# MarioPasc/MU-Diff

Measured on AMD Instinct MI355X. Metric: 256x256 slices/sec (4-step dual-gen reverse), higher is better.
Workload: dtype f32 (convs/attention: fp16 hi+lo split MFMA x3; 3x3 convs that fill the chip: fp16 hi.hi + e4m3 cross terms; fp32 accumulate); 1 GPU; BASELINE config 3 (BraTS-shaped test-split batches of 32; model and slice shapes of config 2): 4-step dual-generator sampling, 256x256, nf=64, ch_mult 1-2-4, 32 slices per GPU per step, batch-sharded over 1 GPU(s), weights replicated; batch=32, hipgraph=True

## Files before the change

include/mudiff_hip.h:

```cpp
#ifndef MUDIFF_HIP_H
#define MUDIFF_HIP_H

#include <stdint.h>

#ifdef __cplusplus
extern "C" {
#endif

#define MUD_OK 0
#define MUD_ERR_ARG 1
#define MUD_ERR_LAUNCH 2
#define MUD_ERR_UNSUPPORTED 3

#define MUD_ACT_NONE 0
#define MUD_ACT_SIGMOID 1
#define MUD_ACT_TANH 2
#define MUD_ACT_SILU 3
#define MUD_ACT_LRELU 4

#define MUD_PRO_NONE 0
#define MUD_PRO_AFFINE 1
#define MUD_PRO_AFFINE_SILU 2
#define MUD_PRO_LRELU 3

// ... 25 lines not shown
  float* out; int ldo;
  int maxdim;
} mud_mlp_args;
int mud_mlp_chain(const mud_mlp_args* a, void* stream);
int mud_mlp_chains(const mud_mlp_args* a, int n, void* stream);

int64_t mud_gn_ws_bytes(int B, int64_t HW, int C, int G);
int mud_gn_scale_shift(const float* x, int B, int64_t HW, int C, int ld, int G, float eps,
                       const float* gamma, const float* beta, int64_t g_bstride,
                       float* scale, float* shift, int ld_ss, float* mean_rstd ,
                       void* ws, void* stream);
int mud_gn_scale_shift_from_sums(const double* sums, int sums_ld, int B, int C, int G, double count, float eps,
                                 const float* gamma, const float* beta, int64_t g_bstride,
                                 float* scale, float* shift, int ld_ss, void* stream);
int mud_channel_mean(const float* x, int B, int64_t HW, int C, int ld, float* out, int ldo, void* ws, void* stream);

typedef struct mud_conv_args {
  const float* x;  int B, H, W, Cin, ldx;
  const void* w;   int64_t w_bstride;
  int ks, stride, pad;
  const float* pro_scale; const float* pro_shift; int pro_ld; int pro_mode;
  const float* bias;
  const float* bias2; int bias2_ld;
  const float* res; int ldr;
  float out_scale; int act;
  const float* emul; int ld_emul;
  const float* egate; int ld_egate;
  const float* eother; int ld_eother;
  float* out; int Cout, ldo;
  int sub2;
  double* stats; int stats_ld;
  int emul_cout;
  const double* gn_sums; int gn_sums_ld;
  int gn_G; float gn_eps; double gn_count;
  const float* gn_gamma; const float* gn_beta;
  int64_t gn_bstride;
  void* splitk_ws; int64_t splitk_ws_bytes;
  unsigned* splitk_counters; int splitk_ncounters;
  const void* skip_w; const float* skip_bias; float* skip_out; int skip_ldo;
  int prec; int w_exp;
} mud_conv_args;

int mud_conv2d_direct(const mud_conv_args* a, void* stream);

int64_t mud_packed_weight_bytes(int ks, int Cin, int Cout);
int mud_pack_weights(const float* src, int64_t s_tap, int64_t s_ci, int64_t s_co, int64_t src_bstride,
                     int ks, int Cin, int Cout, int nbatch, void* dst, void* stream);
int mud_pack_weights_prec(const float* src, int64_t s_tap, int64_t s_ci, int64_t s_co, int64_t src_bstride,
                          int ks, int Cin, int Cout, int nbatch, int prec, int w_exp, void* dst, void* stream);
int64_t mud_packed_weight_bytes_prec(int ks, int Cin, int Cout, int prec);
int mud_conv2d_mfma(const mud_conv_args* a, void* stream);
int mud_conv2d_mfma_prec_supported(const mud_conv_args* a, int prec);
int64_t mud_conv2d_mfma_splitk_bytes(const mud_conv_args* a);

typedef struct mud_census_args {
  const float* x; int B, H, W, C, ldx;
  const float* pro_scale; const float* pro_shift; int pro_ld; int pro_mode;
} mud_census_args;
typedef struct mud_census_out {
  uint64_t n, n_over, n_under, n_fp16_over, amax_bits;
} mud_census_out;
int mud_e4m3_census(const mud_census_args* a, mud_census_out* out, void* stream);

int mud_upfirdn2d(const float* in, int64_t planes, int H, int W, const float* kernel, int kh, int kw,
                  int up_x, int up_y, int down_x, int down_y, int pad_x0, int pad_x1, int pad_y0, int pad_y1,
                  float* out, void* stream);
int mud_fir_nhwc(const float* x, int B, int H, int W, int C, int ldx, const float* kernel_host, int kh, int kw,
                 int up, int down, int pad0, int pad1,
// ... 118 lines not shown
```

mu-diff_amd/backbones/layerspp.py:

```python
import numpy as np
import torch
import torch.nn as nn

from mudiff_hip import ops, precision
from mudiff_hip.ops import (ACT_NONE, ACT_SILU, INV_SQRT2, PRO_AFFINE, PRO_AFFINE_SILU, View)

from . import dense_layer, layers, up_or_down_sampling

conv1x1 = layers.ddpm_conv1x1
conv3x3 = layers.ddpm_conv3x3
NIN = layers.NIN
default_init = layers.default_init
dense = dense_layer.dense

FIR_K = (1, 3, 3, 1)


def _groups(c):
    return min(c // 4, 32)


def use_mfma(cin, cout):
    return cin % 4 == 0 and cin >= 8

# ... 270 lines not shown
        self.dropout = dropout

    def _prepare(self):
        d = dict(c0=ConvParam(self.Conv_0), c1=ConvParam(self.Conv_1))
        if hasattr(self, 'Conv_2'):
            d['c2'] = ConvParam(self.Conv_2)
            if self.up:
                d['c2'].bias = None
                d['c1'].bias = (self.Conv_1.bias.detach() + self.Conv_2.bias.detach()).contiguous()
        return d

    def run(self, x: View, style0, style1, tbias, out: View = None, arena=None):
        if self.dropout and self.training:
            raise NotImplementedError('dropout > 0 in training mode is not part of the inference path')
        p = self.prepared()
        fused = False
        gn0 = self.GroupNorm_0.scale_shift(x, style0)
        sc0, sh0 = (gn0, None) if isinstance(gn0, ops.LazyGN) else gn0
        if self.up:
            kk, up, down, pad = up_or_down_sampling.fir_params('up' if self.fir else 'naive_up', self.fir_kernel)
            h_in, _ = ops.fir_nhwc(x, kk, up, down, pad, pro=(sc0, sh0, PRO_AFFINE_SILU), want_h=True, want_x=False)
            x_skip, _ = ops.fir_nhwc(p['c2'](x), kk, up, down, pad)
            h = p['c0'](h_in, bias2=tbias, arena=arena)
        elif self.down:
            kk, up, down, pad = up_or_down_sampling.fir_params('down' if self.fir else 'naive_down', self.fir_kernel)
            h_in, x_skip = ops.fir_nhwc(x, kk, up, down, pad, pro=(sc0, sh0, PRO_AFFINE_SILU), want_h=True, want_x=True)
            h = p['c0'](h_in, bias2=tbias, arena=arena)
        else:
            x_skip = x
            fused = 'c2' in p and p['c0'].mfma and p['c2'].mfma and ops.fused_skip_ok(x, self.out_ch, PRO_AFFINE_SILU)
            if fused:
                x_skip = View.empty(x.B, x.H, x.W, self.out_ch, x.device)
                h = p['c0'](x, pro=(sc0, sh0, PRO_AFFINE_SILU), bias2=tbias, arena=arena, skip=(p['c2'].w, p['c2'].bias, x_skip))
            else:
                h = p['c0'](x, pro=(sc0, sh0, PRO_AFFINE_SILU), bias2=tbias, arena=arena)
        gn1 = self.GroupNorm_1.scale_shift(h, style1)
        sc1, sh1 = (gn1, None) if isinstance(gn1, ops.LazyGN) else gn1
        if 'c2' in p and not self.up and not fused:
            x_skip = p['c2'](x_skip)
        return p['c1'](h, pro=(sc1, sh1, PRO_AFFINE_SILU), res=x_skip, out_scale=INV_SQRT2 if self.skip_rescale else 1.0, out=out)

    def forward(self, x, temb=None, zemb=None):
        st0 = ops.dense(zemb, self.GroupNorm_0.style.weight.detach(), self.GroupNorm_0.style.bias.detach())
        st1 = ops.dense(zemb, self.GroupNorm_1.style.weight.detach(), self.GroupNorm_1.style.bias.detach())
        tb = None
        if temb is not None:
            tb = ops.dense(temb, self.Dense_0.weight.detach(), self.Dense_0.bias.detach(), act_in=ACT_SILU)
        return self.run(View.from_nchw(x), st0, st1, tb).to_nchw()


class ConvFeatBlock(nn.Module, _Prepared):

    def __init__(self, act, in_ch=None, out_ch=None, zemb_dim=256):
        super().__init__()
        self.conv1 = conv3x3(in_ch, out_ch)
# ... 48 lines not shown
        return self.run(View.from_nchw(x), st).to_nchw()


class ConvBlock_GAP(nn.Module, _Prepared):

    def __init__(self, act, in_ch=None, out_ch=None, zemb_dim=256):
        super().__init__()
        self.conv1 = conv3x3(in_ch, out_ch)
        self.group_norm = GroupNorm_Conv(min(out_ch // 4, 32), out_ch)
        self.act = act
        self.conv2 = conv3x3(out_ch, out_ch)
        self.adaptive_gap = nn.AdaptiveAvgPool2d(1)
        self.fc = dense(out_ch, zemb_dim)

    def _prepare(self):
        return dict(c1=ConvParam(self.conv1), c2=ConvParam(self.conv2))

    def run(self, x: View, arena=None):
        p = self.prepared()
        h = p['c1'](x, arena=arena)
        gn = self.group_norm.scale_shift(h)
        sc, sh = (gn, None) if isinstance(gn, ops.LazyGN) else gn
        h = p['c2'](h, pro=(sc, sh, PRO_AFFINE_SILU))
        gap = ops.channel_mean(h)
        assert gap.shape[1] == self.fc.in_features, f'GAP vector {gap.shape[1]} != fc.in_features {self.fc.in_features}'
        return ops.dense(gap, self.fc.weight.detach(), self.fc.bias.detach())

    def forward(self, x):
        return self.run(View.from_nchw(x))


class GaussianFourierProjection(nn.Module):

    def __init__(self, embedding_size=256, scale=1.0):
# ... 50 lines not shown
```

mu-diff_amd/csrc/conv_direct.hip:

```cpp
#include "mud_common.h"
#include <stdlib.h>

template <int VO, int VI>
__global__ __launch_bounds__(256) void k_conv_direct(mud_conv_args a, int Ho, int Wo, int co_groups) {
  extern __shared__ __attribute__((aligned(16))) char smem_raw[];
  float* st_lds = (float*)smem_raw;
  const int b = blockIdx.y;
  if (a.stats) {
    for (int i = threadIdx.x; i < 2 * a.Cout; i += 256) st_lds[i] = 0.f;
    __syncthreads();
  }
  const unsigned total = (unsigned)Ho * (unsigned)Wo * (unsigned)co_groups;
  const unsigned nthreads = gridDim.x * blockDim.x;
  const unsigned stride = (nthreads / (unsigned)co_groups) * (unsigned)co_groups;
  const unsigned first = blockIdx.x * blockDim.x + threadIdx.x;
  const int cg = (int)(first % (unsigned)co_groups);
  float ssum[VO], ssq[VO];
#pragma unroll
  for (int j = 0; j < VO; ++j) ssum[j] = ssq[j] = 0.f;
  for (uint64_t idx64 = first; first < stride && idx64 < total; idx64 += stride) {
    const unsigned p = (unsigned)idx64 / (unsigned)co_groups;
    const int oy = (int)(p / (unsigned)Wo);
    const int ox = (int)(p - (unsigned)oy * (unsigned)Wo);
    const int co = cg * VO;
// ... 206 lines not shown
      if (a.res) v += a.res[opix * a.ldr + j];
      a.out[opix * a.ldo + j] = mud_act(v * a.out_scale, a.act);
    }
  }
}

extern "C" int mud_conv2d_direct(const mud_conv_args* ap, void* stream) {
  MUD_REQUIRE(ap, "mud_conv2d_direct: null args");
  const mud_conv_args a = *ap;
  MUD_REQUIRE(a.x && a.w && a.out, "mud_conv2d_direct: null pointer");
  MUD_REQUIRE(a.B >= 0 && a.H > 0 && a.W > 0 && a.Cin > 0 && a.Cout > 0 && a.ks >= 1 && a.stride >= 1 && a.pad >= 0,
              "mud_conv2d_direct: bad sizes");
  MUD_REQUIRE(a.ldx >= a.Cin && a.ldo >= a.Cout, "mud_conv2d_direct: ld smaller than C");
  MUD_REQUIRE(a.pro_mode == MUD_PRO_NONE || a.pro_mode == MUD_PRO_LRELU || (a.pro_scale && a.pro_shift && a.pro_ld >= a.Cin), "mud_conv2d_direct: prologue arrays missing");
  MUD_REQUIRE(!a.res || a.ldr >= a.Cout, "mud_conv2d_direct: bad residual view");
  const int Ho = (a.H + 2 * a.pad - a.ks) / a.stride + 1, Wo = (a.W + 2 * a.pad - a.ks) / a.stride + 1;
  MUD_REQUIRE(Ho > 0 && Wo > 0, "mud_conv2d_direct: empty output");
  if (a.B == 0) return MUD_OK;
  const bool vo4 = a.Cout % 4 == 0 && a.ldo % 4 == 0 && mud_aligned16(a.out) && mud_aligned16(a.w) && (a.w_bstride % 16 == 0);
  const bool vi4 = a.Cin % 4 == 0 && a.ldx % 4 == 0 && mud_aligned16(a.x);
  const int co_groups = vo4 ? a.Cout / 4 : a.Cout;
  if (a.Cin == 1 && a.ks == 3 && ((a.stride == 1 && a.pad == 1) || (a.stride == 2 && a.pad == 0)) && vo4 && !a.emul && !a.egate && co_groups <= 256 && a.pro_mode == MUD_PRO_NONE && a.w_bstride == 0 &&
      (!a.res || (a.ldr % 4 == 0 && mud_aligned16(a.res))) && (!a.bias || mud_aligned16(a.bias)) &&
      (!a.bias2 || (a.bias2_ld % 4 == 0 && mud_aligned16(a.bias2)))) {
    MUD_REQUIRE(a.B <= 65535 && (!a.stats || a.stats_ld >= a.Cout), "mud_conv2d_direct: bad batch / stats view");
    const int spb = 256 / co_groups, strips_per_row = (int)mud_cdiv(Wo, HEAD_PIX);
    int64_t blocks = mud_cdiv((int64_t)Ho * strips_per_row, spb);
    if (blocks > 256 * 16) blocks = 256 * 16;
    if (a.stats) {
      static const int cap = getenv("MUD_HEAD_CAP") ? atoi(getenv("MUD_HEAD_CAP")) : 0;
// ... 46 lines not shown
```

mu-diff_amd/csrc/conv_mfma.hip:

```cpp
#include "mud_common.h"
#include <stdlib.h>
#include <type_traits>
#include <utility>

typedef int i32x4 __attribute__((ext_vector_type(4)));
typedef int i32x8 __attribute__((ext_vector_type(8)));
typedef _Float16 f16x4 __attribute__((ext_vector_type(4)));
typedef _Float16 f16x8 __attribute__((ext_vector_type(8)));

typedef mud_h16x4 h16x4;
typedef mud_h16x8 h16x8;
__device__ __forceinline__ int cm_e4m3x4(f32x4 v, float scale) {
  v = v * scale;
#pragma unroll
  for (int e = 0; e < 4; ++e) v[e] = __builtin_amdgcn_fmed3f(v[e], -448.0f, 448.0f);
  int p = __builtin_amdgcn_cvt_pk_fp8_f32(v[0], v[1], 0, false);
  return __builtin_amdgcn_cvt_pk_fp8_f32(v[2], v[3], p, true);
}
#define CM_BN 64
#define CM_BPLANE (CM_BN * 32)
#define CM_BSTEP (2 * CM_BPLANE)
#define CM_PIX 80
#define CM_GN_MAXC 1024
#define CM_GN_BYTES (2 * CM_GN_MAXC * 4)
// ... 320 lines not shown
        *(i32x4*)(smem + loff[j] + 64) = i32x4{0, 0, 0, 0};
        *(i32x4*)(smem + G::BUF + loff[j] + 64) = i32x4{0, 0, 0, 0};
      }
    }
  }
  dma_b(kc0 * G::NG);
  dma_b2(kc0);
  fetch_raw(kc0);

  const int emul_lim = a.emul_cout > 0 ? a.emul_cout : a.Cout;
  const bool vec = ((a.Cout | a.ldo | emul_lim | (a.res ? a.ldr : 0) | (a.emul ? a.ld_emul : 0) | (a.egate ? (a.ld_egate | a.ld_eother) : 0)) & 3) == 0 &&
                   mud_dev_aligned16(a.out) && (!a.res || mud_dev_aligned16(a.res)) && (!a.emul || mud_dev_aligned16(a.emul)) &&
                   (!a.egate || (mud_dev_aligned16(a.egate) && mud_dev_aligned16(a.eother)));
  const bool slab_mode = KS == 3 && nsplit > 1 && fin.counters != nullptr;
  const bool res_in_acc = !DUAL && KS == 3 && a.res != nullptr && !a.sub2 && nsplit == 1;
  if (res_in_acc) {
#pragma unroll
    for (int n = 0; n < 2; ++n) {
      const int co = (nt * WN + wn) * CM_BN + n * 32 + r;
#pragma unroll
      for (int m = 0; m < MT; ++m) {
        const int gy = ty0 + wm * MT + m;
#pragma unroll
        for (int reg = 0; reg < 16; ++reg) {
          const int gx = tx0 + (reg & 3) + 8 * (reg >> 2) + 4 * hh;
          const bool ok = gy < a.H && gx < a.W && co < a.Cout;
          acc[m][n][reg] = ok ? a.res[(((int64_t)b * a.H + gy) * a.W + gx) * a.ldr + co] : 0.f;
        }
      }
    }
  }
// ... 947 lines not shown
  if (a.ks != 3 || a.sub2 || (a.pro_mode != MUD_PRO_NONE && a.pro_mode != MUD_PRO_AFFINE_SILU)) return false;
  if (a.skip_w && a.pro_mode != MUD_PRO_AFFINE_SILU) return false;
  const int v = cm_variant3(a, nullptr);
  return v == CMV_8X2 || v == CMV_16X1 || v == CMV_8X1R;
}
extern "C" int mud_conv2d_mfma_prec_supported(const mud_conv_args* ap, int prec) {
  if (!ap || ap->B <= 0 || ap->H <= 0 || ap->W <= 0 || ap->Cin <= 0 || ap->Cout <= 0) return 0;
  if (prec == MUD_PREC_16X3) return ap->ks == 1 || ap->ks == 3;
  if (prec == MUD_PREC_16X1)
    return ap->ks == 3 && ap->pro_mode >= MUD_PRO_NONE && ap->pro_mode <= MUD_PRO_LRELU && (!ap->skip_w || ap->pro_mode == MUD_PRO_AFFINE_SILU);
  mud_conv_args a = *ap;
  a.prec = prec;
  return prec == MUD_PREC_FP8X && cm_fp8x_built(a);
}

extern "C" int mud_conv2d_mfma(const mud_conv_args* ap, void* stream) {
  MUD_REQUIRE(ap, "mud_conv2d_mfma: null args");
  mud_conv_args a = *ap;
  MUD_REQUIRE(a.x && a.w && a.out, "mud_conv2d_mfma: null pointer");
  MUD_REQUIRE((a.ks == 1 || a.ks == 3) && a.stride == 1 && a.pad == a.ks / 2, "mud_conv2d_mfma: only ks in {1,3}, stride 1, pad ks/2 (got ks=%d stride=%d pad=%d)", a.ks, a.stride, a.pad);
  MUD_REQUIRE(a.B >= 0 && a.H > 0 && a.W > 0 && a.Cin > 0 && a.Cout > 0, "mud_conv2d_mfma: bad sizes");
  MUD_REQUIRE(a.Cin % 4 == 0 && a.ldx % 4 == 0 && a.ldx >= a.Cin && mud_aligned16(a.x), "mud_conv2d_mfma: needs Cin%%4==0 (Cin=%d), ldx%%4==0 (ldx=%d), 16-byte aligned x", a.Cin, a.ldx);
  MUD_REQUIRE((int64_t)a.H * a.W * a.ldx < 0x7fffffffLL, "mud_conv2d_mfma: one image must stay below 2^31 elements");
  MUD_REQUIRE(mud_aligned16(a.w) && a.w_bstride % 16 == 0, "mud_conv2d_mfma: packed weights must be 16-byte aligned");
  MUD_REQUIRE(a.ldo >= a.Cout && (!a.res || a.ldr >= a.Cout), "mud_conv2d_mfma: bad output/residual view");
  MUD_REQUIRE(!a.stats || a.stats_ld >= a.Cout, "mud_conv2d_mfma: bad stats view");
  MUD_REQUIRE(!a.sub2 || (a.ks == 3 && (a.H & 1) && (a.W & 1)), "mud_conv2d_mfma: sub2 needs ks == 3 and odd H, W");
  MUD_REQUIRE(a.emul_cout >= 0 && a.emul_cout <= a.Cout, "mud_conv2d_mfma: emul_cout out of range");
  MUD_REQUIRE((!a.emul || a.ld_emul >= (a.emul_cout > 0 ? a.emul_cout : a.Cout)) && (!a.egate || (a.eother && a.ld_egate >= a.Cout && a.ld_eother >= a.Cout)), "mud_conv2d_mfma: bad emul / egate / eother view");
  MUD_REQUIRE(a.pro_mode >= MUD_PRO_NONE && a.pro_mode <= MUD_PRO_LRELU, "mud_conv2d_mfma: unknown prologue mode %d", a.pro_mode);
// ... 8 lines not shown
    MUD_REQUIRE(a.pro_scale && a.pro_shift && a.pro_ld >= a.Cin && a.pro_ld % 4 == 0 && mud_aligned16(a.pro_scale) && mud_aligned16(a.pro_shift),
                "mud_conv2d_mfma: prologue arrays missing or misaligned");
    MUD_REQUIRE(a.Cin <= CM_GN_MAXC, "mud_conv2d_mfma: a launch with prologue arrays takes Cin <= %d (the kernels keep them in LDS; Cin=%d)", CM_GN_MAXC, a.Cin);
  } else {
    a.pro_scale = a.pro_shift = a.x;
    a.pro_ld = 0;
    a.gn_sums = nullptr;
  }
  if (a.skip_w) {
    MUD_REQUIRE(a.ks == 3 && a.pro_mode == MUD_PRO_AFFINE_SILU && !a.res && !a.sub2 && !a.emul && !a.egate,
                "mud_conv2d_mfma: the fused skip conv needs ks == 3, the AFFINE_SILU prologue and a plain epilogue");
    MUD_REQUIRE(a.skip_out && a.Cin <= 512 && a.Cout % 4 == 0 && a.skip_ldo >= a.Cout && a.skip_ldo % 4 == 0 && a.ldo % 4 == 0 &&
                mud_aligned16(a.skip_w) && mud_aligned16(a.skip_out) && mud_aligned16(a.out),
                "mud_conv2d_mfma: fused skip conv needs Cin <= 512, Cout %% 4 == 0 and aligned float4 output rows (Cin=%d Cout=%d)", a.Cin, a.Cout);
  }
  MUD_REQUIRE(a.prec == MUD_PREC_16X3 || a.prec == MUD_PREC_FP8X || a.prec == MUD_PREC_16X1, "mud_conv2d_mfma: unknown arithmetic plan prec=%d", a.prec);
  MUD_REQUIRE(a.prec != MUD_PREC_16X1 || a.ks == 3, "mud_conv2d_mfma: MUD_PREC_16X1 is built for ks == 3 only (got ks=%d)", a.ks);
  MUD_REQUIRE(a.prec != MUD_PREC_FP8X || (cm_fp8x_built(a) && a.w_exp >= -100 && a.w_exp <= 100),
              "mud_conv2d_mfma: MUD_PREC_FP8X is not built for this launch (ask mud_conv2d_mfma_prec_supported first; the weights were packed for it and cannot be read by another plan)");
  if (a.B == 0) return MUD_OK;
  hipStream_t s = (hipStream_t)stream;
#ifdef MUD_EXPERIMENT_WS
  if (cm_ws_wanted(a)) return cm_ws_dispatch(a, s);
#endif
  if (a.prec == MUD_PREC_FP8X) {
    const int v8 = cm_variant3(a, nullptr);
    if (v8 == CMV_8X1R) return a.pro_mode == MUD_PRO_NONE ? cm_launch_pro<3, 1, 8, 1, MUD_PRO_NONE, false, MUD_PREC_FP8X>(a, s) : cm_launch_pro<3, 1, 8, 1, MUD_PRO_AFFINE_SILU, false, MUD_PREC_FP8X>(a, s);
    const bool x2 = v8 == CMV_8X2;
    if (a.skip_w) return x2 ? cm_launch_pro<3, 2, 4, 2, MUD_PRO_AFFINE_SILU, true, MUD_PREC_FP8X>(a, s) : cm_launch_pro<3, 2, 8, 1, MUD_PRO_AFFINE_SILU, true, MUD_PREC_FP8X>(a, s);
    if (a.pro_mode == MUD_PRO_NONE) return x2 ? cm_launch_pro<3, 2, 4, 2, MUD_PRO_NONE, false, MUD_PREC_FP8X>(a, s) : cm_launch_pro<3, 2, 8, 1, MUD_PRO_NONE, false, MUD_PREC_FP8X>(a, s);
// ... 44 lines not shown
```

mu-diff_amd/mudiff_hip/__init__.py:

```python
from __future__ import annotations

import ctypes as C
import os

import torch

_HERE = os.path.dirname(os.path.abspath(__file__))
_SHIPPED = os.path.join(_HERE, 'libmudiff_hip.so')
_LIB_PATH = os.environ.get('MUDIFF_HIP_LIB', _SHIPPED)
_lib = None
PREC_16X3, PREC_FP8X, PREC_16X1 = 0, 1, 2

ACT_NONE, ACT_SIGMOID, ACT_TANH, ACT_SILU, ACT_LRELU = 0, 1, 2, 3, 4
PRO_NONE, PRO_AFFINE, PRO_AFFINE_SILU, PRO_LRELU = 0, 1, 2, 3


class MudiffHipError(RuntimeError):
    pass


class ConvArgs(C.Structure):
    _fields_ = [
        ('x', C.c_void_p), ('B', C.c_int), ('H', C.c_int), ('W', C.c_int), ('Cin', C.c_int), ('ldx', C.c_int),
        ('w', C.c_void_p), ('w_bstride', C.c_int64),
# ... 2 lines not shown
        ('bias', C.c_void_p),
        ('bias2', C.c_void_p), ('bias2_ld', C.c_int),
        ('res', C.c_void_p), ('ldr', C.c_int),
        ('out_scale', C.c_float), ('act', C.c_int),
        ('emul', C.c_void_p), ('ld_emul', C.c_int), ('egate', C.c_void_p), ('ld_egate', C.c_int), ('eother', C.c_void_p), ('ld_eother', C.c_int),
        ('out', C.c_void_p), ('Cout', C.c_int), ('ldo', C.c_int),
        ('sub2', C.c_int),
        ('stats', C.c_void_p), ('stats_ld', C.c_int),
        ('emul_cout', C.c_int),
        ('gn_sums', C.c_void_p), ('gn_sums_ld', C.c_int), ('gn_G', C.c_int), ('gn_eps', C.c_float), ('gn_count', C.c_double),
        ('gn_gamma', C.c_void_p), ('gn_beta', C.c_void_p), ('gn_bstride', C.c_int64),
        ('splitk_ws', C.c_void_p), ('splitk_ws_bytes', C.c_int64),
        ('splitk_counters', C.c_void_p), ('splitk_ncounters', C.c_int),
        ('skip_w', C.c_void_p), ('skip_bias', C.c_void_p), ('skip_out', C.c_void_p), ('skip_ldo', C.c_int),
        ('prec', C.c_int), ('w_exp', C.c_int),
    ]


MLP_MAX_LAYERS = 6


class MlpArgs(C.Structure):
    _fields_ = [
        ('x', C.c_void_p), ('ldx', C.c_int), ('B', C.c_int),
        ('nlayers', C.c_int), ('dims', C.c_int * (MLP_MAX_LAYERS + 1)),
        ('W', C.c_void_p * MLP_MAX_LAYERS), ('b', C.c_void_p * MLP_MAX_LAYERS),
        ('pixel_norm', C.c_int), ('act', C.c_int), ('act_last', C.c_int),
        ('out', C.c_void_p), ('ldo', C.c_int), ('maxdim', C.c_int),
    ]

# ... 23 lines not shown
_SIGNATURES = {
    'mud_version': (C.c_int, []),
    'mud_last_error': (C.c_char_p, []),
    'mud_build_flags': (C.c_char_p, []),
    'mud_posterior_sample': (_I, [_P, _P, _P, _P, _P, _P, _P, _P, _I, _P, _I, _L, _P]),
    'mud_q_sample': (_I, [_P, _P, _P, _I, _P, _P, _I, _P, _I, _L, _P]),
    'mud_timestep_embedding': (_I, [_P, _P, _I, _I, _F, _P]),
    'mud_pixel_norm': (_I, [_P, _P, _I, _I, _P]),
    'mud_dense': (_I, [_P, _I, _P, _P, _P, _I, _I, _I, _I, _I, _I, _P]),
    'mud_mlp_chain': (_I, [C.POINTER(MlpArgs), _P]),
    'mud_mlp_chains': (_I, [C.POINTER(MlpArgs), _I, _P]),
    'mud_gn_ws_bytes': (_L, [_I, _L, _I, _I]),
    'mud_gn_scale_shift': (_I, [_P, _I, _L, _I, _I, _I, _F, _P, _P, _L, _P, _P, _I, _P, _P, _P]),
    'mud_gn_scale_shift_from_sums': (_I, [_P, _I, _I, _I, _I, C.c_double, _F, _P, _P, _L, _P, _P, _I, _P]),
    'mud_channel_mean': (_I, [_P, _I, _L, _I, _I, _P, _I, _P, _P]),
    'mud_conv2d_direct': (_I, [C.POINTER(ConvArgs), _P]),
    'mud_packed_weight_bytes': (_L, [_I, _I, _I]),
    'mud_pack_weights': (_I, [_P, _L, _L, _L, _L, _I, _I, _I, _I, _P, _P]),
    'mud_pack_weights_prec': (_I, [_P, _L, _L, _L, _L, _I, _I, _I, _I, _I, _I, _P, _P]),
    'mud_packed_weight_bytes_prec': (_L, [_I, _I, _I, _I]),
    'mud_conv2d_mfma': (_I, [C.POINTER(ConvArgs), _P]),
    'mud_conv2d_mfma_prec_supported': (_I, [C.POINTER(ConvArgs), _I]),
    'mud_conv2d_mfma_splitk_bytes': (_L, [C.POINTER(ConvArgs)]),
    'mud_upfirdn2d': (_I, [_P, _L, _I, _I, _P, _I, _I, _I, _I, _I, _I, _I, _I, _I, _I, _P, _P]),
    'mud_fir_nhwc': (_I, [_P, _I, _I, _I, _I, _I, C.POINTER(C.c_float), _I, _I, _I, _I, _I, _I, _P, _P, _I, _I, _P, _I, _P, _I, _P]),
    'mud_minibatch_stddev': (_I, [_P, _I, _L, _I, _I, _I, _P, _P]),
    'mud_attention_supported': (_I, [_I]),
    'mud_attention_ws_bytes': (_L, [_I, _I, _I]),
    'mud_attention': (_I, [_P, _I, _I, _I, _I, _F, _P, _I, _P, _P]),
    'mud_softmax_rows': (_I, [_P, _L, _I, _I, _P]),
    'mud_mul': (_I, [_P, _I, _P, _I, _P, _I, _L, _I, _P]),
    'mud_gate_mix': (_I, [_P, _I, _P, _I, _P, _I, _P, _I, _I, _L, _I, _P, _I, _P]),
    'mud_fourier_embedding': (_I, [_P, _P, _P, _I, _I, _P]),
    'mud_resize_bilinear': (_I, [_P, _L, _I, _I, _I, _I, _P, _P]),
    'mud_affine_clamp': (_I, [_P, _L, _F, _F, _F, _F, _P, _P]),
    'mud_e4m3_census': (_I, [C.POINTER(CensusArgs), _P, _P]),
    'mud_value_range_ws_bytes': (_L, []),
    'mud_value_range': (_I, [_P, _L, _P, _L, _P, _P, _P]),
# ... 95 lines not shown
```

mu-diff_amd/mudiff_hip/ops.py:

```python
from __future__ import annotations

import collections
import ctypes as C
import math
import os

import numpy as np
import torch

from . import (ACT_LRELU, ACT_NONE, ACT_SIGMOID, ACT_SILU, ACT_TANH, PREC_16X1, PREC_16X3, PREC_FP8X, PRO_AFFINE, PRO_AFFINE_SILU, PRO_LRELU,
               PRO_NONE, ConvArgs, MudiffHipError, check, load, ptr, require_gpu)


DETERMINISTIC = os.environ.get('MUD_DETERMINISTIC', '0') == '1'


class StatsArena:

    def __init__(self, device, chunk_doubles=1 << 18):
        self.device, self.chunk = device, chunk_doubles
        self.buf, self.used = None, 0

    def take(self, B, C):
        if DETERMINISTIC:
# ... 317 lines not shown
def conv3x3_would_split_k(x: View, cout):
    a = ConvArgs()
    a.x, a.B, a.H, a.W, a.Cin, a.ldx, a.ks, a.stride, a.pad = x.ptr, x.B, x.H, x.W, x.C, x.ld, 3, 1, 1
    a.out, a.Cout, a.ldo = x.ptr, cout, (cout + 3) & ~3
    return load().mud_conv2d_mfma_splitk_bytes(C.byref(a)) > 0


FUSE_SKIP_SPLIT = os.environ.get('MUD_FUSE_SKIP_SPLIT', '1') != '0'


def fused_skip_ok(x: View, cout, pro_mode):
    return (FUSE_SKIP and pro_mode == PRO_AFFINE_SILU and x.C % 4 == 0 and 8 <= x.C <= 512 and cout % 4 == 0
            and (FUSE_SKIP_SPLIT or not conv3x3_would_split_k(x, cout)))


def resolve_pro(pro):
    if pro is not None and isinstance(pro[0], LazyGN):
        sc, sh = pro[0].tensors()
        return (sc, sh, pro[2])
    return pro


def channel_mean(x: View):
    lib = load()
    HW = x.H * x.W
    ws = _workspace(x.device, lib.mud_gn_ws_bytes(x.B, HW, x.C, x.C))
    out = torch.empty(x.B, x.C, device=x.device, dtype=torch.float32)
    _launch('channel_mean', x.device, lib.mud_channel_mean, x.ptr, x.B, HW, x.C, x.ld, ptr(out), x.C, ptr(ws), STREAM, nbytes=4.0 * x.npix * x.C)
    return out


def pack_weights(src, s_tap, s_ci, s_co, ks, Cin, Cout, nbatch=1, src_bstride=0, src_offset=0, prec=PREC_16X3, w_exp=0):
    lib = load()
    require_gpu(src)
    nbytes = lib.mud_packed_weight_bytes_prec(ks, Cin, Cout, prec)
    if nbytes < 0:
        raise MudiffHipError(f'pack_weights: plan {prec} has no packed form for ks={ks}')
    dst = torch.empty(nbatch, nbytes, device=src.device, dtype=torch.uint8)
    _launch('pack_weights', src.device, lib.mud_pack_weights_prec, C.c_void_p(src.data_ptr() + 4 * src_offset), s_tap, s_ci, s_co, src_bstride, ks, Cin, Cout,
            nbatch, prec, w_exp, ptr(dst), STREAM)
    return dst


# ... 62 lines not shown
    if PREC_PLAN == 'fp16':
        return PREC_16X1 if conv_prec_supported(x, cout, pro_mode, PREC_16X1, skip=skip, sub2=sub2) else PREC_16X3
    if PREC_PLAN != 'all' and not fp8x_pays(x.B, x.H, x.W, x.C, cout):
        return PREC_16X3
    return PREC_FP8X if conv_prec_supported(x, cout, pro_mode, PREC_FP8X, skip=skip, sub2=sub2) else PREC_16X3


Launch = collections.namedtuple('Launch', 'layer ks mfma prec shape sub2 skip pro')


RECORD = None


def conv(x: View, w, ks, Cout, *, mfma, stride=1, pad=None, pro=None, bias=None, bias2=None, res: View = None,
         out_scale=1.0, act=ACT_NONE, out: View = None, w_bstride=0, arena=None, sub2=False, emul: View = None, gate=None, emul_cout=0,
         skip=None, prec=PREC_16X3, w_exp=0, layer=None):
    if RECORD is not None:
        if torch.cuda.is_current_stream_capturing():
            raise RuntimeError('precision.launch_record() is eager only: the launch is being captured into a graph')
        RECORD.append(Launch(layer, ks, bool(mfma), prec, (x.B, x.H, x.W, x.C, Cout), bool(sub2), skip is not None,
                             PRO_NONE if pro is None else pro[2]))
    lib = load()
    pad = ks // 2 if pad is None else pad
    Ho = (x.H + 2 * pad - ks) // stride + 1
    Wo = (x.W + 2 * pad - ks) // stride + 1
    if sub2:
        assert mfma and ks == 3 and stride == 1 and x.H % 2 == 1 and x.W % 2 == 1
        Ho, Wo = x.H // 2, x.W // 2
    if out is None:
        out = View.empty(x.B, Ho, Wo, Cout, x.device, arena)
    assert (out.B, out.H, out.W, out.C) == (x.B, Ho, Wo, Cout), ((out.B, out.H, out.W, out.C), (x.B, Ho, Wo, Cout))
# ... 12 lines not shown
        a.pro_mode = pro[2]
        a.gn_sums, a.gn_sums_ld, a.gn_G, a.gn_eps, a.gn_count = gn.x.stats_ptr, gn.x.stats.shape[1], gn.G, gn.eps, float(gn.x.H * gn.x.W)
        a.gn_gamma, a.gn_beta, a.gn_bstride = ptr(gn.gamma), ptr(gn.beta), gn.bstride
    elif pro is not None:
        sc, sh, mode = pro
        assert sc.shape == (x.B, x.C) and sc.stride(1) == 1 and sh.stride() == sc.stride()
        a.pro_scale, a.pro_shift, a.pro_ld, a.pro_mode = ptr(sc), ptr(sh), sc.stride(0), mode
    else:
        a.pro_mode = PRO_NONE
    if bias is not None:
        assert bias.numel() == Cout and bias.is_contiguous()
        a.bias = ptr(bias)
    if bias2 is not None:
        assert bias2.shape == (x.B, Cout) and bias2.stride(1) == 1
        a.bias2, a.bias2_ld = ptr(bias2), bias2.stride(0)
    if res is not None:
        assert (res.B, res.H, res.W, res.C) == (x.B, Ho, Wo, Cout)
        a.res, a.ldr = res.ptr, res.ld
    a.out_scale, a.act = out_scale, act
    a.sub2 = 1 if sub2 else 0
    if emul is not None:
        assert (emul.B, emul.H, emul.W, emul.C) == (x.B, Ho, Wo, emul_cout or Cout)
        a.emul, a.ld_emul, a.emul_cout = emul.ptr, emul.ld, emul_cout
    if gate is not None:
        gv, ov = gate
        assert (gv.B, gv.H, gv.W, gv.C) == (x.B, Ho, Wo, Cout) == (ov.B, ov.H, ov.W, ov.C)
        a.egate, a.ld_egate, a.eother, a.ld_eother = gv.ptr, gv.ld, ov.ptr, ov.ld
    a.out, a.Cout, a.ldo = out.ptr, Cout, out.ld
    a.prec, a.w_exp = prec, w_exp
    if out.stats is not None:
        a.stats, a.stats_ld = out.stats_ptr, out.stats.shape[1]
# ... 1 lines not shown
    if skip is not None:
        sw, sb, so = skip
        assert mfma and ks == 3 and res is None and (so.B, so.H, so.W, so.C) == (x.B, Ho, Wo, Cout)
        a.skip_w, a.skip_bias, a.skip_out, a.skip_ldo = ptr(sw), ptr(sb), so.ptr, so.ld
        skip_flops = 2.0 * x.B * Ho * Wo * Cout * x.C
    if mfma and ks == 3:
        cnt = splitk_counters(x.device)
        a.splitk_counters, a.splitk_ncounters = ptr(cnt), cnt.numel()
        nws = lib.mud_conv2d_mfma_splitk_bytes(C.byref(a))
        if nws > 0:
            keep = (keep, torch.empty(nws, device=x.device, dtype=torch.uint8))
            a.splitk_ws, a.splitk_ws_bytes = ptr(keep[1]), nws
    fn = lib.mud_conv2d_mfma if mfma else lib.mud_conv2d_direct
    name = (f'conv_mfma_k{ks}' if mfma else f'conv_direct_k{ks}') + {PREC_FP8X: '_fp8x', PREC_16X1: '_fp16'}.get(prec, '')
    flops = 2.0 * x.B * Ho * Wo * Cout * x.C * ks * ks + skip_flops
    nbytes = 4.0 * (x.npix * x.C + out.npix * Cout * ((2 if res is not None else 1) + (1 if skip is not None else 0))) + (w.numel() * w.element_size() if w_bstride == 0 else x.B * w_bstride)
    _launch(name, x.device, fn, C.byref(a), STREAM, flops=flops, nbytes=nbytes)
    return out


CENSUS_FIELDS = ('n', 'n_over', 'n_under', 'n_fp16_over', 'amax_bits')


def new_census_slot(device):
    return torch.zeros(len(CENSUS_FIELDS), device=device, dtype=torch.int64)


def e4m3_census(x: View, pro, out):
    from . import CensusArgs
    require_gpu(x.base, out)
    assert out.dtype == torch.int64 and out.numel() == len(CENSUS_FIELDS) and out.is_contiguous()
# ... 545 lines not shown
```

Baseline: 105.4 slices/s.

## Fuse FIR upsample of skip into conv residual; add GAP style moments kernel

Up-sampling ResBlocks now pass the low-resolution skip tensor straight to the final 3x3 MFMA conv. The conv applies the 4x4 FIR up-sampling stencil inline while loading the residual into the accumulator, which removes a separate FIR pass and the full-resolution intermediate tensor. Separately, a style encoder whose input has one channel now computes GAP(conv2(SiLU(GN(conv1(x))))) in a new three-kernel path built from GN statistics and boundary-corrected moments, without materialising the 64/256-channel feature maps. Both paths are on by default behind env flags, and they add exact-arithmetic reformulations that change rounding order.

Result: no change. 106.2 slices/s (median of 6 runs) (+0.8%).

```diff
diff --git a/include/mudiff_hip.h b/include/mudiff_hip.h
--- a/include/mudiff_hip.h
+++ b/include/mudiff_hip.h
@@ -63,6 +63,10 @@
                                  const float* gamma, const float* beta, int64_t g_bstride,
                                  float* scale, float* shift, int ld_ss, void* stream);
 int mud_channel_mean(const float* x, int B, int64_t HW, int C, int ld, float* out, int ldo, void* ws, void* stream);
+
+int64_t mud_gap_style_ws_bytes(int B, int H, int W, int C);
+int mud_gap_style(const float* x, int B, int H, int W, int ldx, const float* w1, const float* b1, int C, int G, float eps,
+                  const float* w2, const float* b2, float* out, int ldo, void* ws, void* stream);
 
 typedef struct mud_conv_args {
   const float* x;  int B, H, W, Cin, ldx;
@@ -88,6 +92,7 @@
   unsigned* splitk_counters; int splitk_ncounters;
   const void* skip_w; const float* skip_bias; float* skip_out; int skip_ldo;
   int prec; int w_exp;
+  int res_up; float res_up_k[16];
 } mud_conv_args;
 
 int mud_conv2d_direct(const mud_conv_args* a, void* stream);
@@ -101,6 +106,7 @@
 int mud_conv2d_mfma(const mud_conv_args* a, void* stream);
 int mud_conv2d_mfma_prec_supported(const mud_conv_args* a, int prec);
 int64_t mud_conv2d_mfma_splitk_bytes(const mud_conv_args* a);
+int mud_conv2d_mfma_res_up_supported(const mud_conv_args* a);
 
 typedef struct mud_census_args {
   const float* x; int B, H, W, C, ldx;
diff --git a/mu-diff_amd/backbones/layerspp.py b/mu-diff_amd/backbones/layerspp.py
--- a/mu-diff_amd/backbones/layerspp.py
+++ b/mu-diff_amd/backbones/layerspp.py
@@ -308,13 +308,18 @@
         if self.dropout and self.training:
             raise NotImplementedError('dropout > 0 in training mode is not part of the inference path')
         p = self.prepared()
-        fused = False
+        fused, res_up = False, None
         gn0 = self.GroupNorm_0.scale_shift(x, style0)
         sc0, sh0 = (gn0, None) if isinstance(gn0, ops.LazyGN) else gn0
         if self.up:
             kk, up, down, pad = up_or_down_sampling.fir_params('up' if self.fir else 'naive_up', self.fir_kernel)
             h_in, _ = ops.fir_nhwc(x, kk, up, down, pad, pro=(sc0, sh0, PRO_AFFINE_SILU), want_h=True, want_x=False)
-            x_skip, _ = ops.fir_nhwc(p['c2'](x), kk, up, down, pad)
+            x_skip = p['c2'](x)
+            c1_in = View(h_in.base, h_in.B, h_in.H, h_in.W, self.out_ch)
+            if p['c1'].mfma and ops.res_up_ok(c1_in, self.out_ch, kk, up, down, pad):
+                res_up = kk
+            else:
+                x_skip, _ = ops.fir_nhwc(x_skip, kk, up, down, pad)
             h = p['c0'](h_in, bias2=tbias, arena=arena)
         elif self.down:
             kk, up, down, pad = up_or_down_sampling.fir_params('down' if self.fir else 'naive_down', self.fir_kernel)
@@ -332,7 +337,7 @@
         sc1, sh1 = (gn1, None) if isinstance(gn1, ops.LazyGN) else gn1
         if 'c2' in p and not self.up and not fused:
             x_skip = p['c2'](x_skip)
-        return p['c1'](h, pro=(sc1, sh1, PRO_AFFINE_SILU), res=x_skip, out_scale=INV_SQRT2 if self.skip_rescale else 1.0, out=out)
+        return p['c1'](h, pro=(sc1, sh1, PRO_AFFINE_SILU), res=x_skip, res_up=res_up, out_scale=INV_SQRT2 if self.skip_rescale else 1.0, out=out)
 
     def forward(self, x, temb=None, zemb=None):
         st0 = ops.dense(zemb, self.GroupNorm_0.style.weight.detach(), self.GroupNorm_0.style.bias.detach())
@@ -411,10 +416,14 @@
         self.fc = dense(out_ch, zemb_dim)
 
     def _prepare(self):
-        return dict(c1=ConvParam(self.conv1), c2=ConvParam(self.conv2))
+        return dict(c1=ConvParam(self.conv1), c2=ConvParam(self.conv2), w2=self.conv2.weight.detach().float().contiguous())
 
     def run(self, x: View, arena=None):
         p = self.prepared()
+        fp16_plan = ops.PREC_PLAN == 'fp16' and p['c2'].scope is not None
+        if ops.GAP_MOMENTS and not fp16_plan and not p['c1'].mfma and ops.gap_style_supported(x, p['c2'].cout):
+            gap = ops.gap_style(x, p['c1'].w, p['c1'].bias, self.group_norm.num_groups, p['w2'], p['c2'].bias)
+            return ops.dense(gap, self.fc.weight.detach(), self.fc.bias.detach())
         h = p['c1'](x, arena=arena)
         gn = self.group_norm.scale_shift(h)
         sc, sh = (gn, None) if isinstance(gn, ops.LazyGN) else gn
diff --git a/mu-diff_amd/csrc/conv_direct.hip b/mu-diff_amd/csrc/conv_direct.hip
--- a/mu-diff_amd/csrc/conv_direct.hip
+++ b/mu-diff_amd/csrc/conv_direct.hip
@@ -244,6 +244,7 @@
   MUD_REQUIRE(a.ldx >= a.Cin && a.ldo >= a.Cout, "mud_conv2d_direct: ld smaller than C");
   MUD_REQUIRE(a.pro_mode == MUD_PRO_NONE || a.pro_mode == MUD_PRO_LRELU || (a.pro_scale && a.pro_shift && a.pro_ld >= a.Cin), "mud_conv2d_direct: prologue arrays missing");
   MUD_REQUIRE(!a.res || a.ldr >= a.Cout, "mud_conv2d_direct: bad residual view");
+  MUD_REQUIRE(!a.res_up, "mud_conv2d_direct: the up-sampled residual (res_up) is built for mud_conv2d_mfma's 3x3 launches only");
   const int Ho = (a.H + 2 * a.pad - a.ks) / a.stride + 1, Wo = (a.W + 2 * a.pad - a.ks) / a.stride + 1;
   MUD_REQUIRE(Ho > 0 && Wo > 0, "mud_conv2d_direct: empty output");
   if (a.B == 0) return MUD_OK;
diff --git a/mu-diff_amd/csrc/conv_mfma.hip b/mu-diff_amd/csrc/conv_mfma.hip
--- a/mu-diff_amd/csrc/conv_mfma.hip
+++ b/mu-diff_amd/csrc/conv_mfma.hip
@@ -358,7 +358,46 @@
                    (!a.egate || (mud_dev_aligned16(a.egate) && mud_dev_aligned16(a.eother)));
   const bool slab_mode = KS == 3 && nsplit > 1 && fin.counters != nullptr;
   const bool res_in_acc = !DUAL && KS == 3 && a.res != nullptr && !a.sub2 && nsplit == 1;
-  if (res_in_acc) {
+  constexpr bool RES_UP_BUILT = !(MT == 1 && WM == 8);
+  if (RES_UP_BUILT && res_in_acc && a.res_up) {
+    const int Hl = a.H >> 1, Wl = a.W >> 1;
+    const float* rb = a.res + (int64_t)b * Hl * Wl * a.ldr;
+#pragma unroll
+    for (int n = 0; n < 2; ++n) {
+      const int co = (nt * WN + wn) * CM_BN + n * 32 + r;
+      const bool cok = co < a.Cout;
+#pragma unroll
+      for (int m = 0; m < MT; ++m) {
+        const int gy = ty0 + wm * MT + m, ay = gy & 1, iy0 = (gy >> 1) - 1 + ay;
+        const float* kr0 = a.res_up_k + (ay ? 8 : 12);
+        const float* kr1 = a.res_up_k + (ay ? 0 : 4);
+        const float k00e = kr0[3], k01e = kr0[1], k10e = kr1[3], k11e = kr1[1];
+        const float k00o = kr0[2], k01o = kr0[0], k10o = kr1[2], k11o = kr1[0];
+#pragma unroll
+        for (int g4 = 0; g4 < 4; ++g4) {
+          const int gx0 = tx0 + 8 * g4 + 4 * hh, jb = gx0 >> 1;
+          float lo[2][4];
+#pragma unroll
+          for (int dy = 0; dy < 2; ++dy)
+#pragma unroll
+            for (int dx = 0; dx < 4; ++dx) {
+              const int iy = iy0 + dy, ix = jb - 1 + dx;
+              const bool ok = cok && iy >= 0 && iy < Hl && ix >= 0 && ix < Wl;
+              lo[dy][dx] = ok ? rb[(iy * Wl + ix) * a.ldr + co] : 0.f;
+            }
+#pragma unroll
+          for (int e = 0; e < 4; ++e) {
+            const int c0 = (e >> 1) + (e & 1);
+            float v = fmaf((e & 1) ? k00o : k00e, lo[0][c0], 0.f);
+            v = fmaf((e & 1) ? k01o : k01e, lo[0][c0 + 1], v);
+            v = fmaf((e & 1) ? k10o : k10e, lo[1][c0], v);
+            v = fmaf((e & 1) ? k11o : k11e, lo[1][c0 + 1], v);
+            acc[m][n][g4 * 4 + e] = (gy < a.H && gx0 + e < a.W && cok) ? v : 0.f;
+          }
+        }
+      }
+    }
+  } else if (res_in_acc) {
 #pragma unroll
     for (int n = 0; n < 2; ++n) {
       const int co = (nt * WN + wn) * CM_BN + n * 32 + r;
@@ -1336,6 +1375,13 @@
   return prec == MUD_PREC_FP8X && cm_fp8x_built(a);
 }
 
+extern "C" int mud_conv2d_mfma_res_up_supported(const mud_conv_args* ap) {
+  if (!ap || ap->B <= 0 || ap->H <= 0 || ap->W <= 0 || ap->Cin <= 0 || ap->Cout <= 0) return 0;
+  if (ap->ks != 3 || ap->sub2 || ap->skip_w || ap->H % 2 || ap->W % 2) return 0;
+  if (cm_variant3(*ap, nullptr) == CMV_8X1R) return 0;
+  return mud_conv2d_mfma_splitk_bytes(ap) == 0;
+}
+
 extern "C" int mud_conv2d_mfma(const mud_conv_args* ap, void* stream) {
   MUD_REQUIRE(ap, "mud_conv2d_mfma: null args");
   mud_conv_args a = *ap;
@@ -1374,6 +1420,13 @@
                 mud_aligned16(a.skip_w) && mud_aligned16(a.skip_out) && mud_aligned16(a.out),
                 "mud_conv2d_mfma: fused skip conv needs Cin <= 512, Cout %% 4 == 0 and aligned float4 output rows (Cin=%d Cout=%d)", a.Cin, a.Cout);
   }
+  if (a.res_up) {
+    MUD_REQUIRE(a.res && mud_conv2d_mfma_res_up_supported(&a),
+                "mud_conv2d_mfma: the up-sampled residual is built for unsplit 3x3 launches with a residual, even H and W, no sub2, no fused skip conv, "
+                "and not on the one-row 64 -> 64 tile (ask mud_conv2d_mfma_res_up_supported first; ks=%d H=%d W=%d Cin=%d Cout=%d)", a.ks, a.H, a.W, a.Cin, a.Cout);
+    MUD_REQUIRE((int64_t)(a.H / 2) * (a.W / 2) * a.ldr < 0x7fffffffLL, "mud_conv2d_mfma: one low-resolution residual image must stay below 2^31 elements");
+    a.splitk_ws = nullptr;
+  }
   MUD_REQUIRE(a.prec == MUD_PREC_16X3 || a.prec == MUD_PREC_FP8X || a.prec == MUD_PREC_16X1, "mud_conv2d_mfma: unknown arithmetic plan prec=%d", a.prec);
   MUD_REQUIRE(a.prec != MUD_PREC_16X1 || a.ks == 3, "mud_conv2d_mfma: MUD_PREC_16X1 is built for ks == 3 only (got ks=%d)", a.ks);
   MUD_REQUIRE(a.prec != MUD_PREC_FP8X || (cm_fp8x_built(a) && a.w_exp >= -100 && a.w_exp <= 100),
diff --git a/mu-diff_amd/csrc/gap_style.hip b/mu-diff_amd/csrc/gap_style.hip
--- /dev/null
+++ b/mu-diff_amd/csrc/gap_style.hip
@@ -0,0 +1,231 @@
+#include "mud_common.h"
+
+#define GAP_PIX 8
+#define GAP_MAXC 256
+#define GAP_BLOCKS 2048
+
+struct GapGeom { int co_groups, spb, spr, gx, ny, rows, nblk; };
+
+static GapGeom gap_geom(int B, int H, int W, int C) {
+  GapGeom g;
+  g.co_groups = C / 4;
+  g.spb = 256 / g.co_groups;
+  g.spr = (int)mud_cdiv(W, GAP_PIX);
+  g.gx = (int)mud_cdiv(g.spr, g.spb);
+  int ny = GAP_BLOCKS / ((B > 0 ? B : 1) * g.gx);
+  if (ny < 1) ny = 1;
+  if (ny > H) ny = H;
+  g.rows = (int)mud_cdiv(H, ny);
+  g.ny = (int)mud_cdiv(H, g.rows);
+  g.nblk = g.gx * g.ny;
+  return g;
+}
+
+__device__ __forceinline__ double gap_fold(const double* __restrict__ p, int n, int stride) {
+  double s = 0.0;
+  int k = 0;
+  for (; k + 8 <= n; k += 8) {
+    double t[8];
+#pragma unroll
+    for (int j = 0; j < 8; ++j) t[j] = p[(k + j) * stride];
+#pragma unroll
+    for (int j = 0; j < 8; ++j) s += t[j];
+  }
+  for (; k < n; ++k) s += p[k * stride];
+  return s;
+}
+
+extern "C" int64_t mud_gap_style_ws_bytes(int B, int H, int W, int C) {
+  if (B < 0 || H <= 0 || W <= 0 || C <= 0 || C % 4 || C > GAP_MAXC) return -1;
+  const GapGeom g = gap_geom(B, H, W, C);
+  return (int64_t)B * g.nblk * (2 + 9) * C * (int64_t)sizeof(double);
+}
+
+template <bool MOMENTS>
+__global__ __launch_bounds__(256) void k_gap_pass(const float* __restrict__ x, int H, int W, int ldx, const float* __restrict__ w1,
+                                                  const float* __restrict__ b1, int C, int G, float eps, int co_groups, int spr, int rows,
+                                                  const double* __restrict__ part_in, double* __restrict__ part_out) {
+  constexpr int NQ = MOMENTS ? 9 : 2;
+  __shared__ double red[256 * 4];
+  __shared__ double s_sums[MOMENTS ? 2 * GAP_MAXC : 1];
+  __shared__ __attribute__((aligned(16))) float s_ss[MOMENTS ? 2 * GAP_MAXC : 4];
+  const int tid = threadIdx.x, b = blockIdx.z;
+  const int nblk = gridDim.x * gridDim.y, blk = blockIdx.y * gridDim.x + blockIdx.x;
+  const int cg = tid % co_groups, co = cg * 4, spb = 256 / co_groups, ls = tid / co_groups;
+  const int sx = blockIdx.x * spb + ls, x0 = sx * GAP_PIX;
+  const bool active = ls < spb && sx < spr;
+
+  f32x4 sc = {0.f, 0.f, 0.f, 0.f}, sh = {0.f, 0.f, 0.f, 0.f};
+  if (MOMENTS) {
+    for (int i = tid; i < 2 * C; i += 256) {
+      s_sums[i] = gap_fold(part_in + (int64_t)b * nblk * 2 * C + i, nblk, 2 * C);
+    }
+    __syncthreads();
+    const int cpg = C / G;
+    for (int g = tid; g < G; g += 256) {
+      double s = 0.0, q = 0.0;
+      for (int c = g * cpg; c < (g + 1) * cpg; ++c) {
+        s += s_sums[c];
+        q += s_sums[C + c];
+      }
+      const double n = (double)H * (double)W * cpg, mean = s / n;
+      double var = q / n - mean * mean;
+      if (var < 0.0) var = 0.0;
+      const float rstd = (float)(1.0 / sqrt(var + (double)eps)), meanf = (float)mean;
+      for (int c = g * cpg; c < (g + 1) * cpg; ++c) {
+        s_ss[c] = rstd;
+        s_ss[C + c] = 0.0f - meanf * rstd;
+      }
+    }
+    __syncthreads();
+    sc = *(const f32x4*)(s_ss + co);
+    sh = *(const f32x4*)(s_ss + C + co);
+  }
+
+  f32x4 w[9];
+#pragma unroll
+  for (int t = 0; t < 9; ++t) w[t] = *(const f32x4*)(w1 + t * C + co);
+  f32x4 bias = {0.f, 0.f, 0.f, 0.f};
+  if (b1) bias = *(const f32x4*)(b1 + co);
+  const float* xb = x + (int64_t)b * H * W * ldx;
+
+  double acc[NQ][4];
+#pragma unroll
+  for (int q = 0; q < NQ; ++q)
+#pragma unroll
+    for (int e = 0; e < 4; ++e) acc[q][e] = 0.0;
+
+  const int y0 = blockIdx.y * rows, y1 = y0 + rows < H ? y0 + rows : H;
+  const int kl = W - 1 - x0;
+  const bool has_c0 = x0 == 0, has_c1 = kl >= 0 && kl < GAP_PIX;
+  for (int y = y0; active && y < y1; ++y) {
+    float win[3][GAP_PIX + 2];
+#pragma unroll
+    for (int dy = 0; dy < 3; ++dy) {
+      const int iy = y + dy - 1;
+      const bool yok = iy >= 0 && iy < H;
+      const int rowoff = (yok ? iy : 0) * W;
+#pragma unroll
+      for (int j = 0; j < GAP_PIX + 2; ++j) {
+        const int ix = x0 + j - 1;
+        const bool ok = yok && ix >= 0 && ix < W;
+        const float v = xb[(rowoff + (ok ? ix : 0)) * ldx];
+        win[dy][j] = ok ? v : 0.f;
+      }
+    }
+    f32x4 s4 = {0.f, 0.f, 0.f, 0.f}, q4 = {0.f, 0.f, 0.f, 0.f};
+    f32x4 aL = {0.f, 0.f, 0.f, 0.f};
+#pragma unroll
+    for (int k = 0; k < GAP_PIX; ++k) {
+      if (x0 + k >= W) break;
+      f32x4 h = bias;
+#pragma unroll
+      for (int t = 0; t < 9; ++t)
+#pragma unroll
+        for (int e = 0; e < 4; ++e) h[e] = fmaf(win[t / 3][k + t % 3], w[t][e], h[e]);
+      if (MOMENTS) {
+#pragma unroll
+        for (int e = 0; e < 4; ++e) {
+          const float v = mud_silu(fmaf(h[e], sc[e], sh[e]));
+          s4[e] += v;
+          if (k == 0) q4[e] = v;
+          aL[e] = k == kl ? v : aL[e];
+        }
+      } else {
+#pragma unroll
+        for (int e = 0; e < 4; ++e) {
+          s4[e] += h[e];
+          q4[e] = fmaf(h[e], h[e], q4[e]);
+        }
+      }
+    }
+    const bool top = y == 0, bottom = y == H - 1;
+#pragma unroll
+    for (int e = 0; e < 4; ++e) {
+      const double d = (double)s4[e];
+      acc[0][e] += d;
+      if (MOMENTS) {
+        if (top) acc[1][e] += d;
+        if (bottom) acc[2][e] += d;
+        if (has_c0) {
+          const double d0 = (double)q4[e];
+          acc[3][e] += d0;
+          if (top) acc[5][e] += d0;
+          if (bottom) acc[7][e] += d0;
+        }
+        if (has_c1) {
+          const double d1 = (double)aL[e];
+          acc[4][e] += d1;
+          if (top) acc[6][e] += d1;
+          if (bottom) acc[8][e] += d1;
+        }
+      } else {
+        acc[1][e] += (double)q4[e];
+      }
+    }
+  }
+
+  double* out = part_out + ((int64_t)b * nblk + blk) * NQ * C;
+#pragma unroll
+  for (int q = 0; q < NQ; ++q) {
+#pragma unroll
+    for (int e = 0; e < 4; ++e) red[tid * 4 + e] = acc[q][e];
+    __syncthreads();
+    for (int c = tid; c < C; c += 256) {
+      double s = 0.0;
+      for (int l = 0; l < spb; ++l) s += red[(l * co_groups + (c >> 2)) * 4 + (c & 3)];
+      out[q * C + c] = s;
+    }
+    __syncthreads();
+  }
+}
+
+__global__ __launch_bounds__(256) void k_gap_apply(const double* __restrict__ part, int nblk, int C, int H, int W, const float* __restrict__ w2,
+                                                   const float* __restrict__ b2, float* __restrict__ out, int ldo) {
+  __shared__ double prim[9 * GAP_MAXC];
+  __shared__ double M[9 * GAP_MAXC];
+  const int b = blockIdx.x, tid = threadIdx.x, lane = tid & 63, wave = tid >> 6;
+  for (int i = tid; i < 9 * C; i += 256) {
+    prim[i] = gap_fold(part + (int64_t)b * nblk * 9 * C + i, nblk, 9 * C);
+  }
+  __syncthreads();
+  for (int i = tid; i < 9 * C; i += 256) {
+    const int ci = i / 9, t = i - ci * 9, dy = t / 3, dx = t - dy * 3;
+    double m = prim[ci];
+    if (dy != 1) m -= prim[(dy == 0 ? 2 : 1) * C + ci];
+    if (dx != 1) m -= prim[(dx == 0 ? 4 : 3) * C + ci];
+    if (dy != 1 && dx != 1) m += prim[(5 + (dy == 0 ? 2 : 0) + (dx == 0 ? 1 : 0)) * C + ci];
+    M[i] = m;
+  }
+  __syncthreads();
+  const double inv = 1.0 / ((double)H * (double)W);
+  for (int co = wave; co < C; co += 4) {
+    const float* wr = w2 + co * 9 * C;
+    double s = 0.0;
+    for (int i = lane; i < 9 * C; i += 64) s += (double)wr[i] * M[i];
+    s = mud_wave_sum(s);
+    if (lane == 0) out[(int64_t)b * ldo + co] = (float)((b2 ? (double)b2[co] : 0.0) + s * inv);
+  }
+}
+
+extern "C" int mud_gap_style(const float* x, int B, int H, int W, int ldx, const float* w1, const float* b1, int C, int G, float eps,
+                             const float* w2, const float* b2, float* out, int ldo, void* ws, void* stream) {
+  MUD_REQUIRE(x && w1 && w2 && out && ws, "mud_gap_style: null pointer");
+  MUD_REQUIRE(B >= 0 && B <= 65535 && H > 0 && W > 0 && ldx >= 1, "mud_gap_style: bad sizes B=%d H=%d W=%d ldx=%d", B, H, W, ldx);
+  MUD_REQUIRE((int64_t)H * W * ldx < 0x7fffffffLL, "mud_gap_style: one image must stay below 2^31 elements");
+  MUD_REQUIRE(C > 0 && C % 4 == 0 && C <= GAP_MAXC && G > 0 && C % G == 0, "mud_gap_style: needs C%%4==0, C<=%d, C%%G==0 (C=%d, G=%d)", GAP_MAXC, C, G);
+  MUD_REQUIRE(mud_aligned16(w1) && (!b1 || mud_aligned16(b1)) && mud_aligned16(ws) && ldo >= C, "mud_gap_style: w1 / b1 / ws must be 16-byte aligned, ldo >= C");
+  if (B == 0) return MUD_OK;
+  const GapGeom g = gap_geom(B, H, W, C);
+  hipStream_t s = (hipStream_t)stream;
+  double* part1 = (double*)ws;
+  double* part2 = part1 + (int64_t)B * g.nblk * 2 * C;
+  const dim3 grid(g.gx, g.ny, B), block(256);
+  hipLaunchKernelGGL((k_gap_pass<false>), grid, block, 0, s, x, H, W, ldx, w1, b1, C, G, eps, g.co_groups, g.spr, g.rows, (const double*)nullptr, part1);
+  MUD_CHECK_LAUNCH("mud_gap_style(statistics)");
+  hipLaunchKernelGGL((k_gap_pass<true>), grid, block, 0, s, x, H, W, ldx, w1, b1, C, G, eps, g.co_groups, g.spr, g.rows, (const double*)part1, part2);
+  MUD_CHECK_LAUNCH("mud_gap_style(moments)");
+  hipLaunchKernelGGL(k_gap_apply, dim3(B), dim3(256), 0, s, (const double*)part2, g.nblk, C, H, W, w2, b2, out, ldo);
+  MUD_CHECK_LAUNCH("mud_gap_style(apply)");
+  return MUD_OK;
+}
diff --git a/mu-diff_amd/mudiff_hip/__init__.py b/mu-diff_amd/mudiff_hip/__init__.py
--- a/mu-diff_amd/mudiff_hip/__init__.py
+++ b/mu-diff_amd/mudiff_hip/__init__.py
@@ -40,6 +40,7 @@
         ('splitk_counters', C.c_void_p), ('splitk_ncounters', C.c_int),
         ('skip_w', C.c_void_p), ('skip_bias', C.c_void_p), ('skip_out', C.c_void_p), ('skip_ldo', C.c_int),
         ('prec', C.c_int), ('w_exp', C.c_int),
+        ('res_up', C.c_int), ('res_up_k', C.c_float * 16),
     ]
 
 
@@ -93,6 +94,8 @@
     'mud_gn_scale_shift': (_I, [_P, _I, _L, _I, _I, _I, _F, _P, _P, _L, _P, _P, _I, _P, _P, _P]),
     'mud_gn_scale_shift_from_sums': (_I, [_P, _I, _I, _I, _I, C.c_double, _F, _P, _P, _L, _P, _P, _I, _P]),
     'mud_channel_mean': (_I, [_P, _I, _L, _I, _I, _P, _I, _P, _P]),
+    'mud_gap_style_ws_bytes': (_L, [_I, _I, _I, _I]),
+    'mud_gap_style': (_I, [_P, _I, _I, _I, _I, _P, _P, _I, _I, _F, _P, _P, _P, _I, _P, _P]),
     'mud_conv2d_direct': (_I, [C.POINTER(ConvArgs), _P]),
     'mud_packed_weight_bytes': (_L, [_I, _I, _I]),
     'mud_pack_weights': (_I, [_P, _L, _L, _L, _L, _I, _I, _I, _I, _P, _P]),
@@ -101,6 +104,7 @@
     'mud_conv2d_mfma': (_I, [C.POINTER(ConvArgs), _P]),
     'mud_conv2d_mfma_prec_supported': (_I, [C.POINTER(ConvArgs), _I]),
     'mud_conv2d_mfma_splitk_bytes': (_L, [C.POINTER(ConvArgs)]),
+    'mud_conv2d_mfma_res_up_supported': (_I, [C.POINTER(ConvArgs)]),
     'mud_upfirdn2d': (_I, [_P, _L, _I, _I, _P, _I, _I, _I, _I, _I, _I, _I, _I, _I, _I, _P, _P]),
     'mud_fir_nhwc': (_I, [_P, _I, _I, _I, _I, _I, C.POINTER(C.c_float), _I, _I, _I, _I, _I, _I, _P, _P, _I, _I, _P, _I, _P, _I, _P]),
     'mud_minibatch_stddev': (_I, [_P, _I, _L, _I, _I, _I, _P, _P]),
diff --git a/mu-diff_amd/mudiff_hip/ops.py b/mu-diff_amd/mudiff_hip/ops.py
--- a/mu-diff_amd/mudiff_hip/ops.py
+++ b/mu-diff_amd/mudiff_hip/ops.py
@@ -355,6 +355,20 @@
             and (FUSE_SKIP_SPLIT or not conv3x3_would_split_k(x, cout)))
 
 
+RES_UP = os.environ.get('MUD_RES_UP', '1') != '0'
+
+
+def res_up_ok(x: View, cout, kernel2d, up, down, pad):
+    if not (RES_UP and np.shape(kernel2d) == (4, 4) and (up, down, tuple(pad)) == (2, 1, (2, 1)) and x.C % 4 == 0 and x.C >= 8):
+        return False
+    a = ConvArgs()
+    a.x, a.B, a.H, a.W, a.Cin, a.ldx, a.ks, a.stride, a.pad = x.ptr, x.B, x.H, x.W, x.C, x.ld, 3, 1, 1
+    a.out, a.Cout, a.ldo = x.ptr, cout, (cout + 3) & ~3
+    cnt = splitk_counters(x.device)
+    a.splitk_counters, a.splitk_ncounters = ptr(cnt), cnt.numel()
+    return bool(load().mud_conv2d_mfma_res_up_supported(C.byref(a)))
+
+
 def resolve_pro(pro):
     if pro is not None and isinstance(pro[0], LazyGN):
         sc, sh = pro[0].tensors()
@@ -368,6 +382,26 @@
     ws = _workspace(x.device, lib.mud_gn_ws_bytes(x.B, HW, x.C, x.C))
     out = torch.empty(x.B, x.C, device=x.device, dtype=torch.float32)
     _launch('channel_mean', x.device, lib.mud_channel_mean, x.ptr, x.B, HW, x.C, x.ld, ptr(out), x.C, ptr(ws), STREAM, nbytes=4.0 * x.npix * x.C)
+    return out
+
+
+GAP_MOMENTS = os.environ.get('MUD_GAP_MOMENTS', '1') != '0'
+
+
+def gap_style_supported(x: View, C_):
+    return x.C == 1 and load().mud_gap_style_ws_bytes(x.B, x.H, x.W, C_) >= 0
+
+
+def gap_style(x: View, w1, b1, G, w2, b2, eps=1e-6):
+    lib = load()
+    C_ = w2.shape[0]
+    assert x.C == 1 and tuple(w1.shape) == (3, 3, 1, C_) and tuple(w2.shape) == (C_, C_, 3, 3)
+    require_gpu(x.base, w1, b1, w2, b2)
+    w1, w2 = _f32(w1), _f32(w2)
+    ws = _workspace(x.device, lib.mud_gap_style_ws_bytes(x.B, x.H, x.W, C_))
+    out = torch.empty(x.B, C_, device=x.device, dtype=torch.float32)
+    _launch('gap_style', x.device, lib.mud_gap_style, x.ptr, x.B, x.H, x.W, x.ld, ptr(w1), ptr(b1), C_, G, eps, ptr(w2), ptr(b2), ptr(out), C_,
+            ptr(ws), STREAM, flops=2.0 * x.npix * C_ * 9 * 2, nbytes=2 * 4.0 * x.npix)
     return out
 
 
@@ -460,7 +494,7 @@
 
 def conv(x: View, w, ks, Cout, *, mfma, stride=1, pad=None, pro=None, bias=None, bias2=None, res: View = None,
          out_scale=1.0, act=ACT_NONE, out: View = None, w_bstride=0, arena=None, sub2=False, emul: View = None, gate=None, emul_cout=0,
-         skip=None, prec=PREC_16X3, w_exp=0, layer=None):
+         skip=None, prec=PREC_16X3, w_exp=0, layer=None, res_up=None):
     if RECORD is not None:
         if torch.cuda.is_current_stream_capturing():
             raise RuntimeError('precision.launch_record() is eager only: the launch is being captured into a graph')
@@ -503,7 +537,13 @@
     if bias2 is not None:
         assert bias2.shape == (x.B, Cout) and bias2.stride(1) == 1
         a.bias2, a.bias2_ld = ptr(bias2), bias2.stride(0)
-    if res is not None:
+    if res is not None and res_up is not None:
+        k = np.ascontiguousarray(res_up, dtype=np.float32)
+        assert mfma and ks == 3 and not sub2 and skip is None and k.shape == (4, 4)
+        assert Ho % 2 == 0 and Wo % 2 == 0 and (res.B, res.H, res.W, res.C) == (x.B, Ho // 2, Wo // 2, Cout)
+        a.res, a.ldr, a.res_up = res.ptr, res.ld, 1
+        a.res_up_k[:] = k.ravel().tolist()
+    elif res is not None:
         assert (res.B, res.H, res.W, res.C) == (x.B, Ho, Wo, Cout)
         a.res, a.ldr = res.ptr, res.ld
     a.out_scale, a.act = out_scale, act
@@ -535,7 +575,7 @@
     fn = lib.mud_conv2d_mfma if mfma else lib.mud_conv2d_direct
     name = (f'conv_mfma_k{ks}' if mfma else f'conv_direct_k{ks}') + {PREC_FP8X: '_fp8x', PREC_16X1: '_fp16'}.get(prec, '')
     flops = 2.0 * x.B * Ho * Wo * Cout * x.C * ks * ks + skip_flops
-    nbytes = 4.0 * (x.npix * x.C + out.npix * Cout * ((2 if res is not None else 1) + (1 if skip is not None else 0))) + (w.numel() * w.element_size() if w_bstride == 0 else x.B * w_bstride)
+    nbytes = 4.0 * (x.npix * x.C + out.npix * Cout * ((1 if res is None else 1.25 if res_up is not None else 2) + (1 if skip is not None else 0))) + (w.numel() * w.element_size() if w_bstride == 0 else x.B * w_bstride)
     _launch(name, x.device, fn, C.byref(a), STREAM, flops=flops, nbytes=nbytes)
     return out
 
```
